# nkkrnkl/category-agnostic-pose-estimation

Measured on AMD Instinct MI355X. Metric: episodes/sec (1-shot, 256x256, 17kpt) training step, higher is better.
Workload: dtype f32 storage/accumulate, GEMMs as bf16x3 split (3 bf16 MFMAs per product); 1 GPU; configs[1]: 1-shot training step (fwd+loss+bwd+clip+AdamW at learning rate 0, dropout on), 256x256, 17 kpt, ResNet-50 + deformable transformer, 16 episodes x 2 queries per GPU; episodes_per_gpu=16, queries_per_episode=2, image_size=256, global_batch_episodes=16, parallelism=dp1, weights=random init (no checkpoint offline)

## Files before the change

### category-agnostic-pose-estimation_amd/csrc/gemm_group.hip

```cpp
#include "gemm_tile.h"

namespace {

constexpr int GROUP_MAX = CAPE_GEMM_GROUP_MAX;

struct GroupItem {
  const float* A; const float* B; float* C; float* colsum_out;
  int M, N, K, split_k;
  int lda, ldb, ldc, tilesM;
  int tilesN, cN, cH, cW;
  int cC, cKH, cKW, cStride;
  int cPad, cOH, cOW, cO;
  int cDil, pad_;
};

struct GroupArgs {
  int n, single;
  int bstart[GROUP_MAX + 1];
  GroupItem it[GROUP_MAX];
};
static_assert(sizeof(GroupArgs) <= 4096, "the item table travels as kernel arguments");

template <int BM, int BN, int BMODE, int PREC, bool KFULL>
__global__ void __launch_bounds__(256) gemm_group_kernel(const GroupArgs g) {
// ... 1 lines not shown
  int i = 0;
  while (i + 1 < g.n && b >= g.bstart[i + 1]) ++i;
  const GroupItem& q = g.it[i];
  GemmP p;
  p.M = q.M; p.N = q.N; p.K = q.K;
  p.A = q.A; p.lda = q.lda; p.B = q.B; p.ldb = q.ldb; p.C = q.C; p.ldc = q.ldc;
  p.cN = q.cN; p.cH = q.cH; p.cW = q.cW; p.cC = q.cC; p.cKH = q.cKH; p.cKW = q.cKW;
  p.cStride = q.cStride; p.cPad = q.cPad; p.cOH = q.cOH; p.cOW = q.cOW; p.cO = q.cO;
  p.cDil = q.cDil;
  p.cPadX = q.cPad; p.cKHp = q.cKH; p.cKWp = q.cKW; p.cTapH0 = 0; p.cTapHS = 1; p.cTapW0 = 0; p.cTapWS = 1;
  p.scale = nullptr; p.bias = nullptr; p.residual = nullptr; p.ldr = 0;
  p.relu = 0; p.accumulate = 1; p.split_k = q.split_k;
  p.colsum_out = q.colsum_out;
  p.drop_thresh = 0; p.inv_keep = 1.f; p.rng_state = nullptr; p.rng_stream = 0;
  p.tilesM = q.tilesM; p.tilesN = q.tilesN;
  p.Bpack = nullptr; p.mask_src = nullptr; p.ldm = 0; p.mask_scale = 1.f;
  p.bdiv = 1; p.sA0 = p.sA1 = p.sB0 = p.sB1 = p.sC0 = p.sC1 = 0;
  p.res_cols = 0; p.sBias0 = p.sBias1 = 0; p.single = g.single;
  gemm_tile_body<BM, BN, 1, BMODE, true, PREC, KFULL>(p, b - g.bstart[i]);
}

template <int BM, int BMODE>
void launch_group(const GroupArgs& g, int prec, bool kfull, hipStream_t s) {
  const dim3 grid((unsigned)g.bstart[g.n]), block(256);
  if (prec == 1) {
    if (kfull) hipLaunchKernelGGL((gemm_group_kernel<BM, BM, BMODE, 1, true>), grid, block, 0, s, g);
    else hipLaunchKernelGGL((gemm_group_kernel<BM, BM, BMODE, 1, false>), grid, block, 0, s, g);
  } else {
    if (kfull) hipLaunchKernelGGL((gemm_group_kernel<BM, BM, BMODE, 0, true>), grid, block, 0, s, g);
    else hipLaunchKernelGGL((gemm_group_kernel<BM, BM, BMODE, 0, false>), grid, block, 0, s, g);
  }
}

}

extern "C" int cape_gemm_group_f32(const cape_gemm_desc* descs, int n, int tile, cape_stream_t stream) {
  CAPE_REQUIRE(descs != nullptr && n >= 1 && n <= GROUP_MAX, "cape_gemm_group_f32: n=%d must be in 1..%d", n, GROUP_MAX);
  CAPE_REQUIRE(tile == 64 || tile == 128, "cape_gemm_group_f32: tile must be 64 or 128");
  const int b_mode = descs[0].b_mode, prec_in = descs[0].precision, prec = prec_in == 0 ? 0 : 1;
  CAPE_REQUIRE(b_mode == 1 || b_mode == 3, "cape_gemm_group_f32: only the weight-gradient modes (a_mode 1, b_mode 1 or 3) are grouped");
  CAPE_REQUIRE(prec_in >= 0 && prec_in <= 2, "cape_gemm_group_f32: precision must be 0 (fp32), 1 (bf16x3) or 2 (single bf16)");
  auto al16 = [](const void* q) { return (reinterpret_cast<uintptr_t>(q) & 15) == 0; };
  GroupArgs g;
  g.n = n;
  g.single = prec_in == 2;
  bool kfull = true;
  long long blocks = 0;
  for (int i = 0; i < n; ++i) {
    const cape_gemm_desc& d = descs[i];
    CAPE_REQUIRE(d.cDil >= 0, "cape_gemm_group_f32: item %d: negative conv dilation (cDil=%d)", i, d.cDil);
    CAPE_REQUIRE(d.cDil <= 1 || d.cKHp <= 0, "cape_gemm_group_f32: item %d: conv dilation (cDil=%d) cannot be combined with a tap sub-lattice", i, d.cDil);
    CAPE_REQUIRE(d.a_mode == 1 && d.b_mode == b_mode && d.precision == prec_in, "cape_gemm_group_f32: item %d: mixed modes / precisions", i);
    CAPE_REQUIRE(d.M > 0 && d.N > 0 && d.K > 0 && d.A && d.B && d.C, "cape_gemm_group_f32: item %d: empty product or null operand", i);
    CAPE_REQUIRE(d.accumulate && !d.scale && !d.bias && !d.residual && !d.relu && d.dropout_p == 0.f && !d.mask_src && d.batch <= 1,
                 "cape_gemm_group_f32: item %d: grouped products accumulate onto C and take no other epilogue operand", i);
    CAPE_REQUIRE(d.split_k >= 1, "cape_gemm_group_f32: item %d: split_k must be >= 1", i);
    CAPE_REQUIRE(al16(d.A) && al16(d.B) && d.lda % 4 == 0 && d.M % 4 == 0 && d.M >= 4 && d.N % 4 == 0 && d.N >= 4 &&
                     (b_mode == 3 || d.ldb % 4 == 0),
                 "cape_gemm_group_f32: item %d: operands must be 16-byte aligned with M, N, lda, ldb multiples of 4", i);
    CAPE_REQUIRE(d.lda < (1ll << 31) && d.ldb < (1ll << 31) && d.ldc < (1ll << 31), "cape_gemm_group_f32: item %d: leading dimension too large", i);
    if (b_mode == 3) {
      const long long taps = (long long)d.cKH * d.cKW;
      CAPE_REQUIRE(d.cC % 4 == 0 && d.cO % 4 == 0 && d.cStride >= 1 && d.cKH >= 1 && d.cKW >= 1, "cape_gemm_group_f32: item %d: bad conv geometry", i);
      CAPE_REQUIRE(d.N == taps * d.cC && d.K == (long long)d.cN * d.cOH * d.cOW && d.M == d.cO, "cape_gemm_group_f32: item %d: conv-wgrad shape mismatch", i);
    }
    GroupItem& q = g.it[i];
    q.A = d.A; q.B = d.B; q.C = d.C; q.colsum_out = d.colsum_out;
    q.M = d.M; q.N = d.N; q.K = d.K; q.split_k = d.split_k;
    q.lda = (int)d.lda; q.ldb = (int)d.ldb; q.ldc = (int)d.ldc;
    q.tilesM = (d.M + tile - 1) / tile; q.tilesN = (d.N + tile - 1) / tile;
    q.cN = d.cN; q.cH = d.cH; q.cW = d.cW; q.cC = d.cC; q.cKH = d.cKH; q.cKW = d.cKW;
    q.cStride = d.cStride; q.cPad = d.cPad; q.cOH = d.cOH; q.cOW = d.cOW; q.cO = d.cO;
    q.cDil = d.cDil > 0 ? d.cDil : 1; q.pad_ = 0;
    kfull = kfull && (d.K % BK == 0);
    g.bstart[i] = (int)blocks;
    const long long nb = (long long)q.tilesM * q.tilesN * d.split_k;
    blocks += (nb + 7) / 8 * 8;
    CAPE_REQUIRE(blocks < (1ll << 30), "cape_gemm_group_f32: grid too large");
  }
  g.bstart[n] = (int)blocks;
  for (int i = n + 1; i <= GROUP_MAX; ++i) g.bstart[i] = (int)blocks;
  hipStream_t s = as_stream(stream);
  if (tile == 64) { if (b_mode == 1) launch_group<64, 1>(g, prec, kfull, s); else launch_group<64, 3>(g, prec, kfull, s); }
  else { if (b_mode == 1) launch_group<128, 1>(g, prec, kfull, s); else launch_group<128, 3>(g, prec, kfull, s); }
  CAPE_LAUNCH_CHECK("cape_gemm_group_f32");
  return 0;
}
```

### category-agnostic-pose-estimation_amd/hip/functional.py

```python
import contextlib
import ctypes
import os

import torch

from . import lib, ops


class Runtime:
    rng = None
    direct_grad = False
    use_side_stream = os.environ.get("CAPE_SIDE_STREAM", "1") == "1"
    side = None
    on_param_grad = []
    capture_keep = None

    pending = []
    side_dirty = False

    defer_wgrad = os.environ.get("CAPE_DEFER_WGRAD", "1") == "1"
    wgrad_group = int(os.environ.get("CAPE_WGRAD_GROUP", "12"))
    wq = {}
    wq_total = 0
    wq_notify = []
    _final_cb = False

    @classmethod
    def side_stream(cls):
        if cls.side is None:
            cls.side = torch.cuda.Stream()
            cls.side_raw = cls.side.cuda_stream
        return cls.side

    @classmethod
    def join(cls):
        cls.flush_wgrads()
        if cls.side is not None and cls.side_dirty:
            cls.side_dirty = False
            lib.call("cape_stream_join", ctypes.c_void_p(ops.raw_current_stream()), ctypes.c_void_p(cls.side_raw))
            if cls.capture_keep is None:
                cls.pending.clear()

    @classmethod
    def notify(cls, *params):
        if cls.wq_total or cls.wq_notify:
            cls.wq_notify.extend(p for p in params if p is not None)
            return
        for cb in cls.on_param_grad:
            for p in params:
                if p is not None:
                    cb(p)

    @classmethod
    def enqueue_wgrad(cls, desc, keep):
        M, N, K, b_mode = desc.M, desc.N, desc.K, desc.b_mode
        key = (ops.group_tile(M, N, K), b_mode, desc.precision)
        dst = [(desc.C, desc.C + 4 * ((M - 1) * desc.ldc + N))]
        if desc.colsum_out:
            dst.append((desc.colsum_out, desc.colsum_out + 4 * M))
        items = cls.wq.setdefault(key, [])
        if any(lo < e and s < hi for it in items for s, e in it[3] for lo, hi in dst):
            cls._launch_class(key)
        cls.wq[key].append((desc, keep, (M, N, K, 1, b_mode), dst))
        cls.wq_total += 1
        if not cls._final_cb:
            try:
                torch.autograd.Variable._execution_engine.queue_callback(cls.flush_wgrads)
                cls._final_cb = True
            except RuntimeError:
                cls.flush_wgrads()
                return
        if cls.wq_total >= cls.wgrad_group or len(cls.wq[key]) >= lib.GEMM_GROUP_MAX:
            cls._flush()

    @classmethod
    def _launch_class(cls, key):
        items = cls.wq.get(key)
        if not items:
            return
        cls.wq[key] = []
        cls.wq_total -= len(items)
        tile = key[0]
        shapes = [it[2] for it in items]
        for it, sk in zip(items, ops.plan_group_splits([sh[:3] for sh in shapes], tile)):
            it[0].split_k = sk
        with _Side([t for it in items for t in it[1]]):
            for i in range(0, len(items), lib.GEMM_GROUP_MAX):
                ops.gemm_group([it[0] for it in items[i:i + lib.GEMM_GROUP_MAX]], shapes[i:i + lib.GEMM_GROUP_MAX], tile)

# ... 1253 lines not shown
```

### category-agnostic-pose-estimation_amd/hip/ops.py

```python
import ctypes
import math
import os
import weakref

import torch

from . import lib

_F32 = torch.float32


_raw_stream = getattr(torch._C, "_cuda_getCurrentRawStream", None)
_raw_device = getattr(torch._C, "_cuda_getDevice", None)


_side = [None]


def raw_current_stream():
    if _raw_stream is not None and _raw_device is not None:
        return _raw_stream(_raw_device())
    return torch.cuda.current_stream().cuda_stream


# ... 280 lines not shown
        assert _avail(B) >= offB + (K - 1) * d.ldb + N, "gemm: B too small"
    if M > 0:
        assert _avail(C) >= offC + (M - 1) * d.ldc + N, "gemm: C too small"
    if residual is not None:
        assert res_cols % 32 == 0 and 0 <= res_cols <= N
        assert _avail(residual) >= (M - 1) * d.ldr + (res_cols or N), "gemm: residual too small"
    if bias is not None:
        assert _avail(bias) >= N
    if scale is not None:
        assert scale.numel() >= N
    return d, (A, B, C, colsum_out)


def launch_gemm(d):
    if GemmProfiler.enabled:
        e0, e1 = torch.cuda.Event(enable_timing=True), torch.cuda.Event(enable_timing=True)
        st = _stream()
        ext = torch.cuda.ExternalStream(st.value) if _side[0] is not None else None
        e0.record(ext)
        lib.call("cape_gemm_f32", ctypes.byref(d), st)
        e1.record(ext)
        M, N, K, nb = d.M, d.N, d.K, max(d.batch, 1)
        GemmProfiler.records.append((e0, e1, 2.0 * M * N * K * nb, (M, N, K, d.a_mode, d.b_mode, d.split_k, nb),
                                     GemmProfiler.alg_bytes(M, N, K, nb), 1))
        return
    lib.call("cape_gemm_f32", ctypes.byref(d), _stream())


_AUTO_SPLIT_NN = os.environ.get("CAPE_AUTO_SPLIT_NN", "1") == "1" and os.environ.get("CAPE_DETERMINISTIC", "0") != "1"
_PACK_MAX_N = int(os.environ.get("CAPE_PACK_MAX_N", "1000000"))
_GROUP_BIG_MN = int(os.environ.get("CAPE_GROUP_BIG_MN", str(64 * 1024)))


def group_tile(M, N, K):
    return 128 if (M >= 128 and N >= 128 and M * N >= _GROUP_BIG_MN and K >= 4096) else 64


def plan_group_splits(shapes, tile):
    target = 1024 if tile == 64 else 512
    tiles = [((M + tile - 1) // tile) * ((N + tile - 1) // tile) for M, N, K in shapes]
    kt = [(K + 31) // 32 for M, N, K in shapes]
    work = sum(t * k for t, k in zip(tiles, kt))
    per_block = max(8.0, work / float(target))
    out = []
    for k in kt:
        s = int(max(1, min(round(k / per_block), k // 8 if k >= 16 else 1, 64)))
        if s >= 8:
            s = s // 8 * 8
        out.append(s)
    return out


def gemm_group(descs, shapes, tile):
    n = len(descs)
    assert 1 <= n <= lib.GEMM_GROUP_MAX
    arr = (lib.GemmDesc * n)(*descs)
    if GemmProfiler.enabled:
        e0, e1 = torch.cuda.Event(enable_timing=True), torch.cuda.Event(enable_timing=True)
        st = _stream()
        ext = torch.cuda.ExternalStream(st.value) if _side[0] is not None else None
        e0.record(ext)
        lib.call("cape_gemm_group_f32", arr, n, tile, st)
        e1.record(ext)
        fl = sum(2.0 * M * N * K for M, N, K, _, _ in shapes)
        by = sum(GemmProfiler.alg_bytes(M, N, K) for M, N, K, _, _ in shapes)
        GemmProfiler.records.append((e0, e1, fl, ("group", tile, shapes[0][4], n), by, n))
        return
    lib.call("cape_gemm_group_f32", arr, n, tile, _stream())


def colsum(X, M, N, out, ldx=None, accumulate=True, nbatch=1, batch_stride=0):
    _chk(X, "colsum.X", contiguous=False)
# ... 906 lines not shown
```

### category-agnostic-pose-estimation_amd/csrc/attention.hip

```cpp
#include "common.h"

namespace {

constexpr int HD = 32;
constexpr int MAXL = 256;
constexpr int ROWS = 64;

struct AttnP {
  long long ldq, ldk, ldv, ldo;
  long long bsq, bsk, bsv, bso;
  int N, H, Lq, Lk;
  float scale;
  int mask_mode, causal_offset;
  const uint8_t* kpm;
  uint32_t thresh; float inv_keep;
  const uint64_t* rng_state; uint32_t rng_stream;
};

template <int CTRL>
__device__ __forceinline__ float dpp_mov(float v) {
  return __builtin_bit_cast(float, __builtin_amdgcn_update_dpp(0, __builtin_bit_cast(int, v), CTRL, 0xf, 0xf, true));
}
__device__ __forceinline__ float quad_sum(float v) {
  v += dpp_mov<0xB1>(v);
  v += dpp_mov<0x4E>(v);
  return v;
}

__device__ __forceinline__ void stage_rows(float* dst, const float* src, long long ld, int rows) {
  for (int idx = threadIdx.x; idx < rows * 8; idx += blockDim.x) {
    const int r = idx >> 3, c = (idx & 7) * 4;
    *reinterpret_cast<float4*>(dst + r * HD + c) = *reinterpret_cast<const float4*>(src + (long long)r * ld + c);
  }
// ... 271 lines not shown
    }
    av[0] += pd * g0.x; av[1] += pd * g0.y; av[2] += pd * g0.z; av[3] += pd * g0.w;
    av[4] += pd * g1.x; av[5] += pd * g1.y; av[6] += pd * g1.z; av[7] += pd * g1.w;
    const float ds = pe * (dp - Ds[ii]) * p.scale;
    ak[0] += ds * q0.x; ak[1] += ds * q0.y; ak[2] += ds * q0.z; ak[3] += ds * q0.w;
    ak[4] += ds * q1.x; ak[5] += ds * q1.y; ak[6] += ds * q1.z; ak[7] += ds * q1.w;
  }
  }
  if (parts > 1) {
    __syncthreads();
    float* red = smem;
    if (part > 0) {
#pragma unroll
      for (int d = 0; d < 8; ++d) { red[(threadIdx.x) * 16 + d] = ak[d]; red[(threadIdx.x) * 16 + 8 + d] = av[d]; }
    }
    __syncthreads();
    if (part == 0) {
      for (int q = 1; q < parts; ++q) {
#pragma unroll
        for (int d = 0; d < 8; ++d) { ak[d] += red[(q * tpp + tl) * 16 + d]; av[d] += red[(q * tpp + tl) * 16 + 8 + d]; }
      }
    }
  }
  if (live && part == 0) {
    float* dk = dK + (long long)n * p.bsk + (long long)j * p.ldk + h * HD + sub * 8;
    float* dv = dV + (long long)n * p.bsv + (long long)j * p.ldv + h * HD + sub * 8;
    *reinterpret_cast<float4*>(dk) = make_float4(ak[0], ak[1], ak[2], ak[3]);
    *reinterpret_cast<float4*>(dk + 4) = make_float4(ak[4], ak[5], ak[6], ak[7]);
    *reinterpret_cast<float4*>(dv) = make_float4(av[0], av[1], av[2], av[3]);
    *reinterpret_cast<float4*>(dv + 4) = make_float4(av[4], av[5], av[6], av[7]);
  }
}

__global__ void __launch_bounds__(256) attn_softmax_fwd_kernel(const float* __restrict__ S, float* __restrict__ P,
                                                               float* __restrict__ Pd, const AttnP p) {
  const long long row = (long long)blockIdx.x * 4 + (threadIdx.x >> 6);
  const long long rows = (long long)p.N * p.H * p.Lq;
  if (row >= rows) return;
  const int lane = threadIdx.x & 63;
  const int i = (int)(row % p.Lq);
  const int n = (int)(row / ((long long)p.H * p.Lq));
  const float* s = S + row * p.Lk;
  const uint8_t* kp = p.mask_mode >= 2 ? p.kpm + (long long)n * p.Lk : nullptr;
  const float dead = p.mask_mode == 3 ? 0.f : NAN;
  const int jend = p.mask_mode == 1 ? min(p.Lk, i + p.causal_offset + 1) : p.Lk;
  uint64_t seed = 0, step = 0;
  if (p.thresh) { seed = p.rng_state[0]; step = p.rng_state[1]; }
  if (p.Lk <= 256) {
    float v[4];
    bool live[4];
    float m = -INFINITY;
#pragma unroll
    for (int k = 0; k < 4; ++k) {
      const int j = lane + 64 * k;
      live[k] = j < jend && !(kp && kp[j]);
      v[k] = live[k] ? s[j] * p.scale : -INFINITY;
      m = fmaxf(m, v[k]);
    }
    m = wave_max(m);
    float l = 0.f;
#pragma unroll
    for (int k = 0; k < 4; ++k) { v[k] = live[k] ? __expf(v[k] - m) : 0.f; l += v[k]; }
    l = wave_sum(l);
    const float inv = 1.f / l;
#pragma unroll
    for (int k = 0; k < 4; ++k) {
// ... 63 lines not shown
  for (int j = lane; j < p.Lk; j += 64) {
    float g = d[j];
    if (p.thresh) g = cape_keep(seed, step, p.rng_stream, (uint64_t)row * p.Lk + j, p.thresh) ? g * p.inv_keep : 0.f;
    d[j] = p.scale * pr[j] * (g - t);
  }
}

int fill(AttnP& p, long long ldq, long long ldk, long long ldv, long long ldo, const long long* bs, int N, int H, int Lq, int Lk, float scale,
         int mask_mode, int causal_offset, const uint8_t* kpm, float dropout_p, const uint64_t* rng_state,
         uint32_t rng_stream, bool fwd = false) {
  CAPE_REQUIRE(Lq >= 1 && Lk >= 1, "cape_attn: Lq=%d Lk=%d must be positive", Lq, Lk);
  CAPE_REQUIRE((ldq % 4) == 0 && (ldk % 4) == 0 && (ldv % 4) == 0 && (ldo % 4) == 0, "cape_attn: row strides must be multiples of 4");
  CAPE_REQUIRE(mask_mode >= 0 && mask_mode <= 3, "cape_attn: bad mask_mode %d", mask_mode);
  CAPE_REQUIRE(mask_mode < 2 || kpm, "cape_attn: key padding mask missing");
  CAPE_REQUIRE(dropout_p == 0.f || (rng_state && dropout_p < 1.f), "cape_attn: dropout needs rng_state");
  p.ldq = ldq; p.ldk = ldk; p.ldv = ldv; p.ldo = ldo;
  p.bsq = bs[0]; p.bsk = bs[1]; p.bsv = bs[2]; p.bso = bs[3];
  CAPE_REQUIRE((bs[0] % 4) == 0 && (bs[1] % 4) == 0 && (bs[2] % 4) == 0 && (bs[3] % 4) == 0, "cape_attn: batch strides must be multiples of 4");
  p.N = N; p.H = H; p.Lq = Lq; p.Lk = Lk; p.scale = scale;
  p.mask_mode = mask_mode; p.causal_offset = causal_offset; p.kpm = kpm;
  p.thresh = dropout_p > 0.f ? cape_drop_threshold(dropout_p) : 0u;
  p.inv_keep = dropout_p > 0.f ? 1.f / (1.f - dropout_p) : 1.f;
  p.rng_state = rng_state; p.rng_stream = rng_stream;
  return 0;
}

int raise_lds_limit() {
  static bool done = false;
  if (done) return 0;
  const int lim = 96 * 1024;
  hipError_t e = hipFuncSetAttribute(reinterpret_cast<const void*>(attn_fwd_kernel), hipFuncAttributeMaxDynamicSharedMemorySize, lim);
  if (e == hipSuccess) e = hipFuncSetAttribute(reinterpret_cast<const void*>(attn_bwd_dq_kernel), hipFuncAttributeMaxDynamicSharedMemorySize, lim);
  if (e == hipSuccess) e = hipFuncSetAttribute(reinterpret_cast<const void*>(attn_bwd_dkv_kernel), hipFuncAttributeMaxDynamicSharedMemorySize, lim);
  if (e != hipSuccess) return cape_set_error("cape_attn: hipFuncSetAttribute: %s", hipGetErrorString(e));
  done = true;
  return 0;
}

}

extern "C" int cape_attn_fwd(const float* Q, const float* K, const float* V, float* O, float* lse, long long ldq,
                             long long ldk, long long ldv, long long ldo, long long bsq, long long bsk, long long bsv,
                             long long bso, int N, int H, int Lq, int Lk, float scale,
                             int mask_mode, int causal_offset, const uint8_t* kpm, float dropout_p,
                             const uint64_t* rng_state, uint32_t rng_stream, cape_stream_t stream) {
  CAPE_REQUIRE(Q && K && V && O && lse, "cape_attn_fwd: null pointer");
  if (N <= 0 || H <= 0) return 0;
  AttnP p;
  const long long bs[4] = {bsq, bsk, bsv, bso};
  if (fill(p, ldq, ldk, ldv, ldo, bs, N, H, Lq, Lk, scale, mask_mode, causal_offset, kpm, dropout_p, rng_state, rng_stream, true)) return 1;
  if (Lq == 1 && dropout_p == 0.f && Lk <= DEC_MAXL && H <= 65535 && N <= 65535) {
    hipLaunchKernelGGL(attn_decode_kernel, dim3(H, N), dim3(64), 0, as_stream(stream), Q, K, V, O, lse, p);
    CAPE_LAUNCH_CHECK("cape_attn_fwd(decode)");
    return 0;
  }
  if (raise_lds_limit()) return 1;
  CAPE_REQUIRE((Lq + ROWS - 1) / ROWS <= 65535 * 32, "cape_attn_fwd: Lq too large");
  const size_t sh = (size_t)2 * (Lk < MAXL ? Lk : MAXL) * HD * sizeof(float);
  hipLaunchKernelGGL(attn_fwd_kernel, dim3((Lq + ROWS - 1) / ROWS, H, N), dim3(256), sh, as_stream(stream), Q, K, V, O, lse, p);
  CAPE_LAUNCH_CHECK("cape_attn_fwd");
  return 0;
}

extern "C" int cape_attn_bwd(const float* dO, const float* Q, const float* K, const float* V, const float* O,
                             const float* lse, float* dQ, float* dK, float* dV, long long ldq, long long ldk,
                             long long ldv, long long ldo, long long bsq, long long bsk, long long bsv, long long bso,
                             int N, int H, int Lq, int Lk, float scale, int mask_mode, int causal_offset, const uint8_t* kpm, float dropout_p, const uint64_t* rng_state,
                             uint32_t rng_stream, cape_stream_t stream) {
  CAPE_REQUIRE(dO && Q && K && V && O && lse && dQ && dK && dV, "cape_attn_bwd: null pointer");
  if (N <= 0 || H <= 0) return 0;
  AttnP p;
  const long long bs[4] = {bsq, bsk, bsv, bso};
  if (fill(p, ldq, ldk, ldv, ldo, bs, N, H, Lq, Lk, scale, mask_mode, causal_offset, kpm, dropout_p, rng_state, rng_stream)) return 1;
  if (raise_lds_limit()) return 1;
  const int KC = Lk < MAXL ? Lk : MAXL, QC = Lq < MAXL ? Lq : MAXL;
  const size_t sh1 = (size_t)2 * KC * HD * sizeof(float);
  hipLaunchKernelGGL(attn_bwd_dq_kernel, dim3((Lq + ROWS - 1) / ROWS, H, N), dim3(256), sh1, as_stream(stream), dO, Q, K, V,
                     O, lse, dQ, p);
  size_t sh2 = ((size_t)2 * QC * HD + 2 * QC) * sizeof(float);
  if (Lk <= 32 && sh2 < 256 * 16 * sizeof(float)) sh2 = 256 * 16 * sizeof(float);
  hipLaunchKernelGGL(attn_bwd_dkv_kernel, dim3((Lk + ROWS - 1) / ROWS, H, N), dim3(256), sh2, as_stream(stream), dO, Q, K, V,
                     O, lse, dK, dV, p);
  CAPE_LAUNCH_CHECK("cape_attn_bwd");
  return 0;
}

extern "C" int cape_attn_softmax_fwd(const float* S, float* P, float* Pd, int N, int H, int Lq, int Lk, float scale, int mask_mode,
                                     int causal_offset, const uint8_t* kpm, float dropout_p, const uint64_t* rng_state,
                                     uint32_t rng_stream, cape_stream_t stream) {
  CAPE_REQUIRE(S && P, "cape_attn_softmax_fwd: null pointer");
  CAPE_REQUIRE((dropout_p > 0.f) == (Pd != nullptr), "cape_attn_softmax_fwd: Pd goes with dropout");
  if (N <= 0 || H <= 0 || Lq <= 0 || Lk <= 0) return 0;
  AttnP p;
  const long long bs[4] = {0, 0, 0, 0};
  if (fill(p, 4, 4, 4, 4, bs, N, H, Lq, Lk, scale, mask_mode, causal_offset, kpm, dropout_p, rng_state, rng_stream, true)) return 1;
  const long long rows = (long long)N * H * Lq;
  CAPE_REQUIRE((rows + 3) / 4 < (1ll << 31), "cape_attn_softmax_fwd: too many rows");
  hipLaunchKernelGGL(attn_softmax_fwd_kernel, dim3((unsigned)((rows + 3) / 4)), dim3(256), 0, as_stream(stream), S, P, Pd, p);
  CAPE_LAUNCH_CHECK("cape_attn_softmax_fwd");
  return 0;
}

extern "C" int cape_attn_softmax_bwd(const float* P, float* dS, int N, int H, int Lq, int Lk, float scale, float dropout_p,
                                     const uint64_t* rng_state, uint32_t rng_stream, cape_stream_t stream) {
  CAPE_REQUIRE(P && dS, "cape_attn_softmax_bwd: null pointer");
  if (N <= 0 || H <= 0 || Lq <= 0 || Lk <= 0) return 0;
  AttnP p;
// ... 9 lines not shown
```

### category-agnostic-pose-estimation_amd/csrc/common.h

```cpp
#pragma once
#include <hip/hip_runtime.h>
#include <stdint.h>
#include <stdio.h>
#include "../../include/cape_hip.h"

int cape_set_error(const char* fmt, ...);

#define CAPE_REQUIRE(cond, ...)                      \
  do {                                               \
    if (!(cond)) return cape_set_error(__VA_ARGS__); \
  } while (0)

#define CAPE_LAUNCH_CHECK(name)                                                      \
  do {                                                                               \
    hipError_t e_ = hipGetLastError();                                               \
    if (e_ != hipSuccess) return cape_set_error("%s: %s", name, hipGetErrorString(e_)); \
  } while (0)

static inline hipStream_t as_stream(cape_stream_t s) { return (hipStream_t)s; }

__device__ __forceinline__ uint32_t cape_rng_u32(uint64_t seed, uint64_t step, uint32_t stream, uint64_t idx) {
  uint64_t x = seed + 0x9E3779B97F4A7C15ull * (step + 1) + 0xD1342543DE82EF95ull * (uint64_t)(stream + 1);
  x ^= idx * 0xA0761D6478BD642Full;
  x ^= x >> 30; x *= 0xBF58476D1CE4E5B9ull;
  x ^= x >> 27; x *= 0x94D049BB133111EBull;
  x ^= x >> 31;
  return (uint32_t)(x >> 32);
}
__device__ __forceinline__ bool cape_keep(uint64_t seed, uint64_t step, uint32_t stream, uint64_t idx, uint32_t thresh) {
  return cape_rng_u32(seed, step, stream, idx) >= thresh;
}
static inline uint32_t cape_drop_threshold(float p) {
  double t = (double)p * 4294967296.0;
  if (t < 0) t = 0;
  if (t > 4294967295.0) t = 4294967295.0;
  return (uint32_t)t;
}

template <int CTRL>
__device__ __forceinline__ float cape_dpp(float v) {
  return __builtin_bit_cast(float, __builtin_amdgcn_update_dpp(0, __builtin_bit_cast(int, v), CTRL, 0xf, 0xf, true));
}
__device__ __forceinline__ void cape_swap16(float& a, float& b) { asm volatile("s_nop 1\n\tv_permlane16_swap_b32 %0, %1\n\ts_nop 1" : "+v"(a), "+v"(b)); }
__device__ __forceinline__ void cape_swap32(float& a, float& b) { asm volatile("s_nop 1\n\tv_permlane32_swap_b32 %0, %1\n\ts_nop 1" : "+v"(a), "+v"(b)); }
__device__ __forceinline__ float wave_sum(float v) {
  v += cape_dpp<0xB1>(v); v += cape_dpp<0x4E>(v); v += cape_dpp<0x141>(v); v += cape_dpp<0x140>(v);
  float a = v, b = v;
  cape_swap16(a, b);
  v = a + b;
  a = v; b = v;
  cape_swap32(a, b);
  return a + b;
}
__device__ __forceinline__ float wave_max(float v) {
  v = fmaxf(v, cape_dpp<0xB1>(v)); v = fmaxf(v, cape_dpp<0x4E>(v)); v = fmaxf(v, cape_dpp<0x141>(v)); v = fmaxf(v, cape_dpp<0x140>(v));
  float a = v, b = v;
  cape_swap16(a, b);
  v = fmaxf(a, b);
  a = v; b = v;
  cape_swap32(a, b);
// ... 3 lines not shown
```

Measured before the change: 660.0 episodes/s.

## Add 256x256-tile grouped weight-gradient GEMM kernel for large dense products

Adds a 1024-thread grouped GEMM kernel that computes 256x256 output tiles for dense weight-gradient products (b_mode 1, bf16x3 or single bf16). It stages hi/lo bf16 splits in double-buffered LDS with a swizzled transpose layout and uses 32x32x16 MFMAs. The tile selector routes products whose M and N are multiples of 256 and whose K is at least 4096 to this kernel, with a separate split-K block target. The goal is more operand reuse per loaded byte on large wgrad GEMMs. In exchange, each block holds a large LDS footprint, so occupancy is lower, and there are fewer blocks to fill the GPU.

```diff
diff --git a/category-agnostic-pose-estimation_amd/csrc/gemm_group.hip b/category-agnostic-pose-estimation_amd/csrc/gemm_group.hip
--- a/category-agnostic-pose-estimation_amd/csrc/gemm_group.hip
+++ b/category-agnostic-pose-estimation_amd/csrc/gemm_group.hip
@@ -57,14 +57,219 @@
   }
 }
 
+constexpr int W256_PLANE = BK * 256 * 2;
+constexpr int W256_BUF = 4 * W256_PLANE;
+constexpr int W256_LDS = 2 * W256_BUF;
+
+__device__ __forceinline__ int tr_off256(int k, int chunk) { return k * 512 + ((chunk ^ ((k & 3) << 2)) << 4); }
+
+template <bool KFULL, bool SINGLE>
+__global__ void __launch_bounds__(1024) gemm_group_kernel256(const GroupArgs g) {
+  extern __shared__ __attribute__((aligned(16))) char w256_lds[];
+  const int b = blockIdx.x;
+  int it = 0;
+  while (it + 1 < g.n && b >= g.bstart[it + 1]) ++it;
+  const GroupItem& q = g.it[it];
+  const int bid = b - g.bstart[it];
+  const int ntiles = q.tilesM * q.tilesN;
+  if (bid >= ntiles * q.split_k) return;
+  int tile, split;
+  {
+    const int xcd = bid & 7, loc = bid >> 3;
+    if (q.split_k > 1 && (q.split_k & 7) == 0) {
+      split = xcd + 8 * (loc / ntiles);
+      tile = loc % ntiles;
+    } else if (q.split_k > 1) {
+      split = bid / ntiles;
+      tile = bid - split * ntiles;
+    } else {
+      tile = bid;
+      split = 0;
+    }
+  }
+  tile = __builtin_amdgcn_readfirstlane(tile);
+  split = __builtin_amdgcn_readfirstlane(split);
+  const int tm = __builtin_amdgcn_readfirstlane(tile / q.tilesN), tn = tile - tm * q.tilesN;
+  const int m0 = tm * 256, n0 = tn * 256;
+  const int ktiles = (q.K + BK - 1) / BK;
+  const int per = __builtin_amdgcn_readfirstlane((ktiles + q.split_k - 1) / q.split_k);
+  const int kt_begin = split * per;
+  const int kt_end = min(ktiles, kt_begin + per);
+  if (kt_begin >= kt_end) return;
+
+  const int t = threadIdx.x;
+  const int lane = t & 63;
+  const int wave = __builtin_amdgcn_readfirstlane(t >> 6);
+  const int wm = wave >> 2, wn = wave & 3;
+
+  const float* Ag = q.A + m0;
+  const float* Bg = q.B + n0;
+  const int lda = q.lda, ldb = q.ldb, K = q.K;
+  const unsigned lane4 = 4u * lane;
+  int st_off[2];
+#pragma unroll
+  for (int j = 0; j < 2; ++j) st_off[j] = tr_off256(2 * wave + j, lane >> 1) + 8 * (lane & 1);
+  float4 ra[2], rb[2];
+  auto load_tiles = [&](int kt) {
+#pragma unroll
+    for (int j = 0; j < 2; ++j) {
+      const int k = kt * BK + 2 * wave + j;
+      const bool kin = KFULL || k < K;
+      const long long kr = kin ? k : 0;
+      const float4 va = *reinterpret_cast<const float4*>(Ag + kr * lda + lane4);
+      const float4 vb = *reinterpret_cast<const float4*>(Bg + kr * ldb + lane4);
+      ra[j] = kin ? va : zero4();
+      rb[j] = kin ? vb : zero4();
+    }
+  };
+  auto store_tiles = [&](int buf) {
+    char* base = w256_lds + buf * W256_BUF;
+#pragma unroll
+    for (int j = 0; j < 2; ++j) {
+      unsigned h0, l0, h1, l1;
+      split2(ra[j].x, ra[j].y, h0, l0);
+      split2(ra[j].z, ra[j].w, h1, l1);
+      *reinterpret_cast<uint2*>(base + st_off[j]) = make_uint2(h0, h1);
+      *reinterpret_cast<uint2*>(base + W256_PLANE + st_off[j]) = make_uint2(l0, l1);
+      split2(rb[j].x, rb[j].y, h0, l0);
+      split2(rb[j].z, rb[j].w, h1, l1);
+      *reinterpret_cast<uint2*>(base + 2 * W256_PLANE + st_off[j]) = make_uint2(h0, h1);
+      *reinterpret_cast<uint2*>(base + 3 * W256_PLANE + st_off[j]) = make_uint2(l0, l1);
+    }
+  };
+  const bool do_colsum = q.colsum_out != nullptr && tn == 0;
+  float4 csum = zero4();
+  auto colsum_tile = [&]() {
+#pragma unroll
+    for (int j = 0; j < 2; ++j) { csum.x += ra[j].x; csum.y += ra[j].y; csum.z += ra[j].z; csum.w += ra[j].w; }
+  };
+
+  f32x16 acc[2][2];
+#pragma unroll
+  for (int i = 0; i < 2; ++i)
+#pragma unroll
+    for (int j = 0; j < 2; ++j)
+#pragma unroll
+      for (int r = 0; r < 16; ++r) acc[i][j][r] = 0.f;
+
+  const int tr_h = lane >> 5, tr_c = (lane >> 4) & 1, tr_q = (lane >> 2) & 3, tr_p = lane & 3;
+  int fa[2], fb[2];
+#pragma unroll
+  for (int i = 0; i < 2; ++i) {
+    fa[i] = tr_off256(8 * tr_h + tr_q, ((wm * 64 + 32 * i) >> 3) + 2 * tr_c + (tr_p >> 1)) + 8 * (tr_p & 1);
+    fb[i] = tr_off256(8 * tr_h + tr_q, ((wn * 64 + 32 * i) >> 3) + 2 * tr_c + (tr_p >> 1)) + 8 * (tr_p & 1) + 2 * W256_PLANE;
+  }
+  auto compute = [&](int buf, int ks) {
+    const char* base = w256_lds + buf * W256_BUF + ks * (16 * 512);
+    bf16x8 ahi[2], alo[2];
+#pragma unroll
+    for (int i = 0; i < 2; ++i) {
+      ahi[i] = tr_read8(base + fa[i], 4 * 512);
+      if constexpr (!SINGLE) alo[i] = tr_read8(base + fa[i] + W256_PLANE, 4 * 512);
+    }
+#pragma unroll
+    for (int j = 0; j < 2; ++j) {
+      const bf16x8 bhi = tr_read8(base + fb[j], 4 * 512);
+      bf16x8 blo;
+      if constexpr (!SINGLE) blo = tr_read8(base + fb[j] + W256_PLANE, 4 * 512);
+#pragma unroll
+      for (int i = 0; i < 2; ++i) {
+        if constexpr (!SINGLE) {
+          acc[i][j] = __builtin_amdgcn_mfma_f32_32x32x16_bf16(alo[i], bhi, acc[i][j], 0, 0, 0);
+          acc[i][j] = __builtin_amdgcn_mfma_f32_32x32x16_bf16(ahi[i], blo, acc[i][j], 0, 0, 0);
+        }
+        acc[i][j] = __builtin_amdgcn_mfma_f32_32x32x16_bf16(ahi[i], bhi, acc[i][j], 0, 0, 0);
+      }
+    }
+  };
+
+  load_tiles(kt_begin);
+  if (do_colsum) colsum_tile();
+  store_tiles(0);
+  if (kt_begin + 1 < kt_end) load_tiles(kt_begin + 1);
+  __syncthreads();
+  int cur = 0;
+  for (int kt = kt_begin; kt < kt_end; ++kt) {
+    compute(cur, 0);
+    if (kt + 1 < kt_end) {
+      if (do_colsum) colsum_tile();
+      store_tiles(cur ^ 1);
+      if (kt + 2 < kt_end) load_tiles(kt + 2);
+    }
+    compute(cur, 1);
+    __syncthreads();
+    cur ^= 1;
+  }
+
+  const int ln = __builtin_amdgcn_mbcnt_hi(~0u, __builtin_amdgcn_mbcnt_lo(~0u, 0u));
+  if (do_colsum) {
+    float4* red = reinterpret_cast<float4*>(w256_lds);
+    red[wave * 64 + ln] = csum;
+    __syncthreads();
+    if (wave == 0) {
+      float4 r = red[ln];
+#pragma unroll
+      for (int i = 1; i < 16; ++i) { const float4 u = red[ln + 64 * i]; r.x += u.x; r.y += u.y; r.z += u.z; r.w += u.w; }
+      float* cs = q.colsum_out + m0 + 4 * ln;
+      atomicAdd(cs, r.x); atomicAdd(cs + 1, r.y); atomicAdd(cs + 2, r.z); atomicAdd(cs + 3, r.w);
+    }
+  }
+
+  const int ldc = q.ldc;
+  const bool atomic = q.split_k > 1;
+  const unsigned lo = (unsigned)(4 * (ln >> 5) * ldc + (ln & 31));
+#pragma unroll
+  for (int i = 0; i < 2; ++i) {
+#pragma unroll
+    for (int j = 0; j < 2; ++j) {
+      float* c0 = q.C + (long long)(m0 + wm * 64 + i * 32) * ldc + (n0 + wn * 64 + j * 32);
+      if (atomic) {
+#pragma unroll
+        for (int r = 0; r < 16; ++r) atomicAdd(c0 + (lo + (unsigned)(((r & 3) + 8 * (r >> 2)) * ldc)), acc[i][j][r]);
+      } else {
+        float xv[16];
+#pragma unroll
+        for (int r = 0; r < 16; ++r) xv[r] = c0[lo + (unsigned)(((r & 3) + 8 * (r >> 2)) * ldc)];
+#pragma unroll
+        for (int r = 0; r < 16; ++r) c0[lo + (unsigned)(((r & 3) + 8 * (r >> 2)) * ldc)] = acc[i][j][r] + xv[r];
+      }
+    }
+  }
+}
+
+void launch_wgrad256(const GroupArgs& g, bool kfull, hipStream_t s) {
+  const dim3 grid((unsigned)g.bstart[g.n]), block(1024);
+  if (g.single) {
+    if (kfull) hipLaunchKernelGGL((gemm_group_kernel256<true, true>), grid, block, W256_LDS, s, g);
+    else hipLaunchKernelGGL((gemm_group_kernel256<false, true>), grid, block, W256_LDS, s, g);
+  } else {
+    if (kfull) hipLaunchKernelGGL((gemm_group_kernel256<true, false>), grid, block, W256_LDS, s, g);
+    else hipLaunchKernelGGL((gemm_group_kernel256<false, false>), grid, block, W256_LDS, s, g);
+  }
+}
+
+int wgrad256_opt_in() {
+  static bool done = false;
+  if (done) return 0;
+  const void* fns[4] = {reinterpret_cast<const void*>(gemm_group_kernel256<true, false>), reinterpret_cast<const void*>(gemm_group_kernel256<false, false>),
+                        reinterpret_cast<const void*>(gemm_group_kernel256<true, true>), reinterpret_cast<const void*>(gemm_group_kernel256<false, true>)};
+  hipError_t e = hipSuccess;
+  for (int i = 0; i < 4 && e == hipSuccess; ++i) e = hipFuncSetAttribute(fns[i], hipFuncAttributeMaxDynamicSharedMemorySize, W256_LDS);
+  if (e != hipSuccess) return cape_set_error("cape_gemm_group_f32: hipFuncSetAttribute: %s", hipGetErrorString(e));
+  done = true;
+  return 0;
+}
+
 }
 
 extern "C" int cape_gemm_group_f32(const cape_gemm_desc* descs, int n, int tile, cape_stream_t stream) {
   CAPE_REQUIRE(descs != nullptr && n >= 1 && n <= GROUP_MAX, "cape_gemm_group_f32: n=%d must be in 1..%d", n, GROUP_MAX);
-  CAPE_REQUIRE(tile == 64 || tile == 128, "cape_gemm_group_f32: tile must be 64 or 128");
+  CAPE_REQUIRE(tile == 64 || tile == 128 || tile == 256, "cape_gemm_group_f32: tile must be 64, 128 or 256");
   const int b_mode = descs[0].b_mode, prec_in = descs[0].precision, prec = prec_in == 0 ? 0 : 1;
   CAPE_REQUIRE(b_mode == 1 || b_mode == 3, "cape_gemm_group_f32: only the weight-gradient modes (a_mode 1, b_mode 1 or 3) are grouped");
   CAPE_REQUIRE(prec_in >= 0 && prec_in <= 2, "cape_gemm_group_f32: precision must be 0 (fp32), 1 (bf16x3) or 2 (single bf16)");
+  CAPE_REQUIRE(tile != 256 || (b_mode == 1 && prec_in >= 1),
+               "cape_gemm_group_f32: tile 256 takes dense products (b_mode 1) at precision 1 (bf16x3) or 2 (single bf16) only");
   auto al16 = [](const void* q) { return (reinterpret_cast<uintptr_t>(q) & 15) == 0; };
   GroupArgs g;
   g.n = n;
@@ -84,6 +289,8 @@
                      (b_mode == 3 || d.ldb % 4 == 0),
                  "cape_gemm_group_f32: item %d: operands must be 16-byte aligned with M, N, lda, ldb multiples of 4", i);
     CAPE_REQUIRE(d.lda < (1ll << 31) && d.ldb < (1ll << 31) && d.ldc < (1ll << 31), "cape_gemm_group_f32: item %d: leading dimension too large", i);
+    CAPE_REQUIRE(tile != 256 || (d.M % 256 == 0 && d.N % 256 == 0 && d.ldc < (1ll << 26)),
+                 "cape_gemm_group_f32: item %d: tile 256 needs M and N multiples of 256 (M=%d N=%d)", i, d.M, d.N);
     if (b_mode == 3) {
       const long long taps = (long long)d.cKH * d.cKW;
       CAPE_REQUIRE(d.cC % 4 == 0 && d.cO % 4 == 0 && d.cStride >= 1 && d.cKH >= 1 && d.cKW >= 1, "cape_gemm_group_f32: item %d: bad conv geometry", i);
@@ -105,8 +312,10 @@
   }
   g.bstart[n] = (int)blocks;
   for (int i = n + 1; i <= GROUP_MAX; ++i) g.bstart[i] = (int)blocks;
+  if (wgrad256_opt_in()) return 1;
   hipStream_t s = as_stream(stream);
-  if (tile == 64) { if (b_mode == 1) launch_group<64, 1>(g, prec, kfull, s); else launch_group<64, 3>(g, prec, kfull, s); }
+  if (tile == 256) launch_wgrad256(g, kfull, s);
+  else if (tile == 64) { if (b_mode == 1) launch_group<64, 1>(g, prec, kfull, s); else launch_group<64, 3>(g, prec, kfull, s); }
   else { if (b_mode == 1) launch_group<128, 1>(g, prec, kfull, s); else launch_group<128, 3>(g, prec, kfull, s); }
   CAPE_LAUNCH_CHECK("cape_gemm_group_f32");
   return 0;
diff --git a/category-agnostic-pose-estimation_amd/hip/functional.py b/category-agnostic-pose-estimation_amd/hip/functional.py
--- a/category-agnostic-pose-estimation_amd/hip/functional.py
+++ b/category-agnostic-pose-estimation_amd/hip/functional.py
@@ -54,7 +54,7 @@
     @classmethod
     def enqueue_wgrad(cls, desc, keep):
         M, N, K, b_mode = desc.M, desc.N, desc.K, desc.b_mode
-        key = (ops.group_tile(M, N, K), b_mode, desc.precision)
+        key = (ops.group_tile(M, N, K, b_mode, desc.precision), b_mode, desc.precision)
         dst = [(desc.C, desc.C + 4 * ((M - 1) * desc.ldc + N))]
         if desc.colsum_out:
             dst.append((desc.colsum_out, desc.colsum_out + 4 * M))
diff --git a/category-agnostic-pose-estimation_amd/hip/ops.py b/category-agnostic-pose-estimation_amd/hip/ops.py
--- a/category-agnostic-pose-estimation_amd/hip/ops.py
+++ b/category-agnostic-pose-estimation_amd/hip/ops.py
@@ -336,12 +336,20 @@
 _GROUP_BIG_MN = int(os.environ.get("CAPE_GROUP_BIG_MN", str(64 * 1024)))
 
 
-def group_tile(M, N, K):
+GROUP_TILE256 = os.environ.get("CAPE_GROUP_TILE256", "1") == "1"
+_GROUP_TILE256_MINK = int(os.environ.get("CAPE_GROUP_TILE256_MINK", "4096"))
+_GROUP_TARGET256 = int(os.environ.get("CAPE_GROUP_TARGET256", "256"))
+
+
+def group_tile(M, N, K, b_mode=1, precision=None):
+    precision = GEMM_PRECISION if precision is None else precision
+    if GROUP_TILE256 and b_mode == 1 and precision in (1, 2) and M % 256 == 0 and N % 256 == 0 and K >= _GROUP_TILE256_MINK:
+        return 256
     return 128 if (M >= 128 and N >= 128 and M * N >= _GROUP_BIG_MN and K >= 4096) else 64
 
 
 def plan_group_splits(shapes, tile):
-    target = 1024 if tile == 64 else 512
+    target = 1024 if tile == 64 else 512 if tile == 128 else _GROUP_TARGET256
     tiles = [((M + tile - 1) // tile) * ((N + tile - 1) // tile) for M, N, K in shapes]
     kt = [(K + 31) // 32 for M, N, K in shapes]
     work = sum(t * k for t, k in zip(tiles, kt))
```

New measurement: 624.6 episodes/s. -5.4%, worse.

## Add specialized small-Lk attention forward and fused backward kernels

Applied to the files above, without the earlier changes.

Adds dedicated kernels for attention with at most 32 keys. The forward keeps all scores in registers and computes the mask and dropout bits once per row using DPP. The backward fuses the dQ and dK/dV passes into one block per (head, batch), which stages K/V once and reduces the per-slice partial dK/dV in LDS. The intent is to cut launch count, redundant K/V staging and per-element RNG overhead for small key sets such as the keypoint queries. It adds a getenv check on every call, and one block per head/batch may underuse the GPU when N*H is small.

```diff
diff --git a/category-agnostic-pose-estimation_amd/csrc/attention.hip b/category-agnostic-pose-estimation_amd/csrc/attention.hip
--- a/category-agnostic-pose-estimation_amd/csrc/attention.hip
+++ b/category-agnostic-pose-estimation_amd/csrc/attention.hip
@@ -1,4 +1,5 @@
 #include "common.h"
+#include <stdlib.h>
 
 namespace {
 
@@ -336,6 +337,238 @@
   }
 }
 
+constexpr int SK = 32;
+constexpr int SLD = 36;
+constexpr int SDS = 33;
+constexpr int SBT = 512;
+constexpr int SQC = 208;
+constexpr int SRED = 529;
+
+template <int CTRL>
+__device__ __forceinline__ uint32_t dpp_mov_u32(uint32_t v) {
+  return (uint32_t)__builtin_amdgcn_update_dpp(0, (int)v, CTRL, 0xf, 0xf, true);
+}
+
+__global__ void __launch_bounds__(256) attn_small_fwd_kernel(const float* __restrict__ Q, const float* __restrict__ K,
+                                                              const float* __restrict__ V, float* __restrict__ O,
+                                                              float* __restrict__ lse, const AttnP p) {
+  __shared__ __attribute__((aligned(16))) float Ks[SK * HD];
+  __shared__ __attribute__((aligned(16))) float Vs[SK * HD];
+  const int n = blockIdx.z, h = blockIdx.y;
+  const int sub = threadIdx.x & 3;
+  const int i = blockIdx.x * ROWS + (threadIdx.x >> 2);
+  const bool live = i < p.Lq;
+  float q[8], acc[8];
+#pragma unroll
+  for (int d = 0; d < 8; ++d) { q[d] = 0.f; acc[d] = 0.f; }
+  if (live) {
+    const float* qp = Q + (long long)n * p.bsq + (long long)i * p.ldq + h * HD + sub * 8;
+    const float4 a = *reinterpret_cast<const float4*>(qp), b = *reinterpret_cast<const float4*>(qp + 4);
+    q[0] = a.x * p.scale; q[1] = a.y * p.scale; q[2] = a.z * p.scale; q[3] = a.w * p.scale;
+    q[4] = b.x * p.scale; q[5] = b.y * p.scale; q[6] = b.z * p.scale; q[7] = b.w * p.scale;
+  }
+  stage_rows(Ks, K + (long long)n * p.bsk + h * HD, p.ldk, p.Lk);
+  stage_rows(Vs, V + (long long)n * p.bsv + h * HD, p.ldv, p.Lk);
+  uint32_t valid = p.Lk >= 32 ? 0xffffffffu : (1u << p.Lk) - 1u;
+  if (p.mask_mode >= 2) {
+    const int lane = threadIdx.x & 63;
+    valid &= ~(uint32_t)__ballot(lane < p.Lk && p.kpm[(long long)n * p.Lk + lane] != 0);
+  }
+  if (p.mask_mode == 1) {
+    const int c = i + p.causal_offset + 1;
+    valid &= c <= 0 ? 0u : (c >= 32 ? 0xffffffffu : (1u << c) - 1u);
+  }
+  if (!live) valid = 0u;
+  uint32_t keep = 0xffffffffu;
+  if (p.thresh) {
+    const uint64_t base = cape_rng_base(p.rng_state[0], p.rng_state[1], p.rng_stream);
+    const uint64_t rbase = (((uint64_t)n * p.H + h) * p.Lq + (uint64_t)(live ? i : 0)) * p.Lk;
+    uint64_t a = (rbase + sub) * CAPE_RNG_IDX_MUL;
+    uint32_t bits = 0u;
+#pragma unroll
+    for (int t = 0; t < SK / 4; ++t) {
+      if (4 * t < p.Lk) {
+        bits |= (cape_rng_finish(base ^ a) >= p.thresh ? 1u : 0u) << (4 * t + sub);
+        a += 4 * CAPE_RNG_IDX_MUL;
+      }
+    }
+    bits |= dpp_mov_u32<0xB1>(bits);
+    bits |= dpp_mov_u32<0x4E>(bits);
+    keep = bits;
+  }
+  __syncthreads();
+  float s[SK];
+  float m = -INFINITY;
+#pragma unroll
+  for (int j = 0; j < SK; ++j) {
+    s[j] = -INFINITY;
+    if (j < p.Lk) {
+      const float4 k0v = *reinterpret_cast<const float4*>(Ks + j * HD + sub * 8);
+      const float4 k1v = *reinterpret_cast<const float4*>(Ks + j * HD + sub * 8 + 4);
+      const float d = quad_sum(dot8(q, k0v, k1v));
+      s[j] = ((valid >> j) & 1u) ? d : -INFINITY;
+      m = fmaxf(m, s[j]);
+    }
+  }
+  float l = 0.f;
+#pragma unroll
+  for (int j = 0; j < SK; ++j) {
+    if (j < p.Lk) {
+      const float pe = ((valid >> j) & 1u) ? __expf(s[j] - m) : 0.f;
+      l += pe;
+      const float pd = ((keep >> j) & 1u) ? pe * p.inv_keep : 0.f;
+      const float4 v0 = *reinterpret_cast<const float4*>(Vs + j * HD + sub * 8);
+      const float4 v1 = *reinterpret_cast<const float4*>(Vs + j * HD + sub * 8 + 4);
+      acc[0] += pd * v0.x; acc[1] += pd * v0.y; acc[2] += pd * v0.z; acc[3] += pd * v0.w;
+      acc[4] += pd * v1.x; acc[5] += pd * v1.y; acc[6] += pd * v1.z; acc[7] += pd * v1.w;
+    }
+  }
+  if (!live) return;
+  float* op = O + (long long)n * p.bso + (long long)i * p.ldo + h * HD + sub * 8;
+  if (p.mask_mode == 3 && l == 0.f) {
+    *reinterpret_cast<float4*>(op) = make_float4(0.f, 0.f, 0.f, 0.f);
+    *reinterpret_cast<float4*>(op + 4) = make_float4(0.f, 0.f, 0.f, 0.f);
+    if (sub == 0) lse[((long long)n * p.H + h) * p.Lq + i] = 0.f;
+  } else {
+    const float inv = 1.f / l;
+    *reinterpret_cast<float4*>(op) = make_float4(acc[0] * inv, acc[1] * inv, acc[2] * inv, acc[3] * inv);
+    *reinterpret_cast<float4*>(op + 4) = make_float4(acc[4] * inv, acc[5] * inv, acc[6] * inv, acc[7] * inv);
+    if (sub == 0) lse[((long long)n * p.H + h) * p.Lq + i] = m + __logf(l);
+  }
+}
+
+__global__ void __launch_bounds__(SBT) attn_small_bwd_kernel(const float* __restrict__ dO, const float* __restrict__ Q,
+                                                              const float* __restrict__ K, const float* __restrict__ V,
+                                                              const float* __restrict__ O, const float* __restrict__ lse,
+                                                              float* __restrict__ dQ, float* __restrict__ dK, float* __restrict__ dV,
+                                                              const AttnP p, const int qcap, const int qg_floats) {
+  extern __shared__ __attribute__((aligned(16))) float smem[];
+  float* Ks = smem;
+  float* Vs = Ks + SK * SLD;
+  float* Qs = Vs + SK * SLD;
+  float* Gs = Qs + qcap * SLD;
+  float* dSs = Qs + qg_floats;
+  float* Ds = dSs + qcap * SDS;
+  float* Ls = Ds + qcap;
+  const int h = blockIdx.x, n = blockIdx.y, tid = threadIdx.x;
+  const int Lk = p.Lk;
+  for (int idx = tid; idx < Lk * 8; idx += SBT) {
+    const int r = idx >> 3, c = (idx & 7) * 4;
+    *reinterpret_cast<float4*>(Ks + r * SLD + c) = *reinterpret_cast<const float4*>(K + (long long)n * p.bsk + (long long)r * p.ldk + h * HD + c);
+    *reinterpret_cast<float4*>(Vs + r * SLD + c) = *reinterpret_cast<const float4*>(V + (long long)n * p.bsv + (long long)r * p.ldv + h * HD + c);
+  }
+  __syncthreads();
+  const int nsl = SBT / Lk;
+  const int sl = tid / Lk, j = tid - sl * Lk;
+  const bool active = sl < nsl;
+  float ks[HD], v[HD], ak[HD], av[HD];
+#pragma unroll
+  for (int c = 0; c < HD; c += 4) {
+    const float4 a = *reinterpret_cast<const float4*>(Ks + j * SLD + c), b = *reinterpret_cast<const float4*>(Vs + j * SLD + c);
+    ks[c] = a.x * p.scale; ks[c + 1] = a.y * p.scale; ks[c + 2] = a.z * p.scale; ks[c + 3] = a.w * p.scale;
+    v[c] = b.x; v[c + 1] = b.y; v[c + 2] = b.z; v[c + 3] = b.w;
+  }
+#pragma unroll
+  for (int c = 0; c < HD; ++c) { ak[c] = 0.f; av[c] = 0.f; }
+  const bool keymasked = p.mask_mode >= 2 && p.kpm[(long long)n * Lk + j] != 0;
+  uint64_t base = 0;
+  if (p.thresh) base = cape_rng_base(p.rng_state[0], p.rng_state[1], p.rng_stream);
+  const uint64_t astep = (uint64_t)(nsl * Lk) * CAPE_RNG_IDX_MUL;
+  const uint64_t row0 = ((uint64_t)n * p.H + h) * p.Lq;
+  for (int qb = 0; qb < p.Lq; qb += qcap) {
+    const int qc = min(qcap, p.Lq - qb);
+    if (qb) __syncthreads();
+    for (int idx = tid; idx < qc * 8; idx += SBT) {
+      const int r = idx >> 3, c = (idx & 7) * 4;
+      const long long orow = (long long)n * p.bso + (long long)(qb + r) * p.ldo + h * HD + c;
+      const float4 g = *reinterpret_cast<const float4*>(dO + orow), o = *reinterpret_cast<const float4*>(O + orow);
+      *reinterpret_cast<float4*>(Qs + r * SLD + c) = *reinterpret_cast<const float4*>(Q + (long long)n * p.bsq + (long long)(qb + r) * p.ldq + h * HD + c);
+      *reinterpret_cast<float4*>(Gs + r * SLD + c) = g;
+      float d = quad_sum(g.x * o.x + g.y * o.y + g.z * o.z + g.w * o.w);
+      d += dpp_mov<0x141>(d);
+      if ((idx & 7) == 0) { Ds[r] = d; Ls[r] = lse[row0 + qb + r]; }
+    }
+    __syncthreads();
+    if (active) {
+      uint64_t a = ((row0 + qb + sl) * Lk + j) * CAPE_RNG_IDX_MUL;
+      for (int i = sl; i < qc; i += nsl, a += astep) {
+        float q[HD], g[HD];
+#pragma unroll
+        for (int c = 0; c < HD; c += 4) {
+          const float4 x = *reinterpret_cast<const float4*>(Qs + i * SLD + c), y = *reinterpret_cast<const float4*>(Gs + i * SLD + c);
+          q[c] = x.x; q[c + 1] = x.y; q[c + 2] = x.z; q[c + 3] = x.w;
+          g[c] = y.x; g[c + 1] = y.y; g[c + 2] = y.z; g[c + 3] = y.w;
+        }
+        float s4[4] = {0.f, 0.f, 0.f, 0.f}, d4[4] = {0.f, 0.f, 0.f, 0.f};
+#pragma unroll
+        for (int c = 0; c < HD; ++c) { s4[c & 3] += ks[c] * q[c]; d4[c & 3] += v[c] * g[c]; }
+        const float s = (s4[0] + s4[1]) + (s4[2] + s4[3]);
+        float dp = (d4[0] + d4[1]) + (d4[2] + d4[3]);
+        const bool on = !keymasked && !(p.mask_mode == 1 && j > qb + i + p.causal_offset);
+        const float pe = on ? __expf(s - Ls[i]) : 0.f;
+        float pd = pe;
+        if (p.thresh) {
+          const bool keep = cape_rng_finish(base ^ a) >= p.thresh;
+          pd = keep ? pe * p.inv_keep : 0.f;
+          dp = keep ? dp * p.inv_keep : 0.f;
+        }
+        const float ds = on ? pe * (dp - Ds[i]) * p.scale : 0.f;
+#pragma unroll
+        for (int c = 0; c < HD; ++c) { av[c] += pd * g[c]; ak[c] += ds * q[c]; }
+        dSs[i * SDS + j] = ds;
+      }
+    }
+    __syncthreads();
+    for (int r = tid >> 2; r < qc; r += SBT / 4) {
+      const int sub = tid & 3;
+      float acc[8];
+#pragma unroll
+      for (int d = 0; d < 8; ++d) acc[d] = 0.f;
+      for (int jj = 0; jj < Lk; ++jj) {
+        const float ds = dSs[r * SDS + jj];
+        const float4 k0 = *reinterpret_cast<const float4*>(Ks + jj * SLD + sub * 8);
+        const float4 k1 = *reinterpret_cast<const float4*>(Ks + jj * SLD + sub * 8 + 4);
+        acc[0] += ds * k0.x; acc[1] += ds * k0.y; acc[2] += ds * k0.z; acc[3] += ds * k0.w;
+        acc[4] += ds * k1.x; acc[5] += ds * k1.y; acc[6] += ds * k1.z; acc[7] += ds * k1.w;
+      }
+      float* dp_ = dQ + (long long)n * p.bsq + (long long)(qb + r) * p.ldq + h * HD + sub * 8;
+      *reinterpret_cast<float4*>(dp_) = make_float4(acc[0], acc[1], acc[2], acc[3]);
+      *reinterpret_cast<float4*>(dp_ + 4) = make_float4(acc[4], acc[5], acc[6], acc[7]);
+    }
+  }
+  float* red = Qs;
+#pragma unroll
+  for (int rd = 0; rd < HD / 8; ++rd) {
+    if (rd) __syncthreads();
+    if (active) {
+#pragma unroll
+      for (int d = 0; d < 8; ++d) { red[d * SRED + tid] = ak[rd * 8 + d]; red[(8 + d) * SRED + tid] = av[rd * 8 + d]; }
+    }
+    __syncthreads();
+    if (tid < 16 * Lk) {
+      const int d = tid / Lk, jj = tid - d * Lk;
+      float part[8] = {0.f, 0.f, 0.f, 0.f, 0.f, 0.f, 0.f, 0.f};
+      const float* rp = red + d * SRED + jj;
+      int s2 = 0;
+      for (; s2 + 8 <= nsl; s2 += 8) {
+#pragma unroll
+        for (int e = 0; e < 8; ++e) part[e] += rp[(s2 + e) * Lk];
+      }
+#pragma unroll
+      for (int e = 0; e < 8; ++e) if (s2 + e < nsl) part[e] += rp[(s2 + e) * Lk];
+      const float sum = ((part[0] + part[1]) + (part[2] + part[3])) + ((part[4] + part[5]) + (part[6] + part[7]));
+      if (d < 8) dK[(long long)n * p.bsk + (long long)jj * p.ldk + h * HD + rd * 8 + d] = sum;
+      else dV[(long long)n * p.bsv + (long long)jj * p.ldv + h * HD + rd * 8 + d - 8] = sum;
+    }
+  }
+}
+
+bool small_form(int N, int H, int Lk) {
+  if (Lk > SK || N > 65535 || H > 65535) return false;
+  const char* e = getenv("CAPE_ATTN_SMALL");
+  return !(e && e[0] == '0' && e[1] == 0);
+}
+
 __global__ void __launch_bounds__(256) attn_softmax_fwd_kernel(const float* __restrict__ S, float* __restrict__ P,
                                                                float* __restrict__ Pd, const AttnP p) {
   const long long row = (long long)blockIdx.x * 4 + (threadIdx.x >> 6);
@@ -465,6 +698,7 @@
   hipError_t e = hipFuncSetAttribute(reinterpret_cast<const void*>(attn_fwd_kernel), hipFuncAttributeMaxDynamicSharedMemorySize, lim);
   if (e == hipSuccess) e = hipFuncSetAttribute(reinterpret_cast<const void*>(attn_bwd_dq_kernel), hipFuncAttributeMaxDynamicSharedMemorySize, lim);
   if (e == hipSuccess) e = hipFuncSetAttribute(reinterpret_cast<const void*>(attn_bwd_dkv_kernel), hipFuncAttributeMaxDynamicSharedMemorySize, lim);
+  if (e == hipSuccess) e = hipFuncSetAttribute(reinterpret_cast<const void*>(attn_small_bwd_kernel), hipFuncAttributeMaxDynamicSharedMemorySize, lim);
   if (e != hipSuccess) return cape_set_error("cape_attn: hipFuncSetAttribute: %s", hipGetErrorString(e));
   done = true;
   return 0;
@@ -489,6 +723,11 @@
   }
   if (raise_lds_limit()) return 1;
   CAPE_REQUIRE((Lq + ROWS - 1) / ROWS <= 65535 * 32, "cape_attn_fwd: Lq too large");
+  if (small_form(N, H, Lk)) {
+    hipLaunchKernelGGL(attn_small_fwd_kernel, dim3((Lq + ROWS - 1) / ROWS, H, N), dim3(256), 0, as_stream(stream), Q, K, V, O, lse, p);
+    CAPE_LAUNCH_CHECK("cape_attn_fwd(small)");
+    return 0;
+  }
   const size_t sh = (size_t)2 * (Lk < MAXL ? Lk : MAXL) * HD * sizeof(float);
   hipLaunchKernelGGL(attn_fwd_kernel, dim3((Lq + ROWS - 1) / ROWS, H, N), dim3(256), sh, as_stream(stream), Q, K, V, O, lse, p);
   CAPE_LAUNCH_CHECK("cape_attn_fwd");
@@ -506,6 +745,14 @@
   const long long bs[4] = {bsq, bsk, bsv, bso};
   if (fill(p, ldq, ldk, ldv, ldo, bs, N, H, Lq, Lk, scale, mask_mode, causal_offset, kpm, dropout_p, rng_state, rng_stream)) return 1;
   if (raise_lds_limit()) return 1;
+  if (small_form(N, H, Lk)) {
+    const int qcap = Lq < SQC ? Lq : SQC;
+    const int qg = 2 * qcap * SLD > 16 * SRED ? 2 * qcap * SLD : 16 * SRED;
+    const size_t sh = ((size_t)2 * SK * SLD + qg + (size_t)qcap * (SDS + 2)) * sizeof(float);
+    hipLaunchKernelGGL(attn_small_bwd_kernel, dim3(H, N), dim3(SBT), sh, as_stream(stream), dO, Q, K, V, O, lse, dQ, dK, dV, p, qcap, qg);
+    CAPE_LAUNCH_CHECK("cape_attn_bwd(small)");
+    return 0;
+  }
   const int KC = Lk < MAXL ? Lk : MAXL, QC = Lq < MAXL ? Lq : MAXL;
   const size_t sh1 = (size_t)2 * KC * HD * sizeof(float);
   hipLaunchKernelGGL(attn_bwd_dq_kernel, dim3((Lq + ROWS - 1) / ROWS, H, N), dim3(256), sh1, as_stream(stream), dO, Q, K, V,
diff --git a/category-agnostic-pose-estimation_amd/csrc/common.h b/category-agnostic-pose-estimation_amd/csrc/common.h
--- a/category-agnostic-pose-estimation_amd/csrc/common.h
+++ b/category-agnostic-pose-estimation_amd/csrc/common.h
@@ -19,13 +19,18 @@
 
 static inline hipStream_t as_stream(cape_stream_t s) { return (hipStream_t)s; }
 
-__device__ __forceinline__ uint32_t cape_rng_u32(uint64_t seed, uint64_t step, uint32_t stream, uint64_t idx) {
-  uint64_t x = seed + 0x9E3779B97F4A7C15ull * (step + 1) + 0xD1342543DE82EF95ull * (uint64_t)(stream + 1);
-  x ^= idx * 0xA0761D6478BD642Full;
+constexpr uint64_t CAPE_RNG_IDX_MUL = 0xA0761D6478BD642Full;
+__device__ __forceinline__ uint64_t cape_rng_base(uint64_t seed, uint64_t step, uint32_t stream) {
+  return seed + 0x9E3779B97F4A7C15ull * (step + 1) + 0xD1342543DE82EF95ull * (uint64_t)(stream + 1);
+}
+__device__ __forceinline__ uint32_t cape_rng_finish(uint64_t x) {
   x ^= x >> 30; x *= 0xBF58476D1CE4E5B9ull;
   x ^= x >> 27; x *= 0x94D049BB133111EBull;
   x ^= x >> 31;
   return (uint32_t)(x >> 32);
+}
+__device__ __forceinline__ uint32_t cape_rng_u32(uint64_t seed, uint64_t step, uint32_t stream, uint64_t idx) {
+  return cape_rng_finish(cape_rng_base(seed, step, stream) ^ (idx * CAPE_RNG_IDX_MUL));
 }
 __device__ __forceinline__ bool cape_keep(uint64_t seed, uint64_t step, uint32_t stream, uint64_t idx, uint32_t thresh) {
   return cape_rng_u32(seed, step, stream, idx) >= thresh;
```

Result: no change. 647.9 episodes/s before, 647.2 episodes/s after (-0.1%).
